# pytorch/ao

Hardware: NVIDIA H100
Metric: tok/s Llama-3-8B int4-wo (tile_packed_to_4d, g=32) linear stack, decode (higher is better)
Workload: dtype int4 weights -> bf16 MMA (f32 accumulate)

## Files before the change

### ao_b200/csrc/int4_linear.cu

```cuda
#include <cuda_bf16.h>
#include <stdlib.h>

#include "common.h"
#include "ptx.cuh"
#include "ts_gemm.cuh"

namespace ao {
namespace int4k {

using tsg::KCHUNK;
using tsg::ROWS;

__device__ __forceinline__ uint32_t deq_pair(uint32_t magic_bits, __nv_bfloat162 s2, __nv_bfloat162 z2) {
  const __nv_bfloat162 c136 = __floats2bfloat162_rn(136.f, 136.f);
  __nv_bfloat162 v = *reinterpret_cast<__nv_bfloat162*>(&magic_bits);
  v = __hsub2(v, c136);
  v = __hfma2(v, s2, z2);
  return *reinterpret_cast<uint32_t*>(&v);
}

struct Int4Fmt {
  static constexpr bool SS = false;
  static constexpr bool DECODE_2CTA = true;
  static constexpr bool PROMOTE = false;
  static constexpr int X_ELEM_BYTES = 2;
  static constexpr int W_BYTES = ROWS * KCHUNK / 2;
  static constexpr int AUX_BYTES = 2048;
  static constexpr int EPI = tsg::EPI_FLOAT;
  static constexpr int ACC_EXP2 = 0;
  static constexpr int MAX_N_MMA = 128;
  static int make_maps(const int32_t* qdata, const uint16_t* sz, int N, int K, int g, CUtensorMap* tm_w,
                       CUtensorMap* tm_sz) {
    const int KT = K / 128;
    {
      const uint64_t dims[3] = {32, (uint64_t)4 * KT, (uint64_t)N / 8};
      const uint64_t str[2] = {128, (uint64_t)KT * 512};
      const uint32_t box[3] = {32, 4, 16};
      int rc = make_tmap(tm_w, CU_TENSOR_MAP_DATA_TYPE_INT32, 3, qdata, dims, str, box, CU_TENSOR_MAP_SWIZZLE_128B);
      if (rc) return rc;
    }
    const int gpc = g <= 128 ? 128 / g : 1;
    const uint64_t dims[2] = {(uint64_t)N, (uint64_t)K / g};
    const uint64_t str[1] = {(uint64_t)N * 4};
    const uint32_t box[2] = {128, (uint32_t)gpc};
    return make_tmap(tm_sz, CU_TENSOR_MAP_DATA_TYPE_UINT32, 2, sz, dims, str, box, CU_TENSOR_MAP_SWIZZLE_NONE);
  }
  __device__ static __forceinline__ uint32_t w_tx_bytes(const tsg::Params& p) {
    const int gpc = p.group_size <= KCHUNK ? KCHUNK / p.group_size : 1;
    return W_BYTES + gpc * 512;
  }
  __device__ static __forceinline__ void issue_w(const CUtensorMap* tm_w, const CUtensorMap* tm_sz,
                                                 const tsg::Params& p, uint8_t* w_dst, uint8_t* aux_dst,
                                                 uint64_t* bar, int n_tile, int kc, uint64_t policy) {
    tma_load_3d(w_dst, tm_w, bar, 0, 4 * kc, n_tile * (ROWS / 8), policy);
    tma_load_2d(aux_dst, tm_sz, bar, n_tile * ROWS, (kc * KCHUNK) / p.group_size, policy);
  }
  struct Raw {
    uint4 v[2];
    uint32_t sz[2][4];
  };
  __device__ static __forceinline__ void load(const tsg::Params& p, uint32_t w_smem, uint32_t aux_smem, int row_lo,
                                              int lane, Raw& raw) {
    const int gshift = p.group_size == 32 ? 0 : (p.group_size == 64 ? 1 : 2);
#pragma unroll
    for (int h = 0; h < 2; ++h) {
      const int r = row_lo + 8 * h;
      const uint32_t off = (uint32_t)(r >> 3) * 512u + (uint32_t)lane * 16u;
      raw.v[h] = tsg::lds128(w_smem + (off ^ (((off >> 7) & 7) << 4)));
#pragma unroll
      for (int w = 0; w < 4; ++w) raw.sz[h][w] = tsg::lds32(aux_smem + r * 4 + (w >> gshift) * 512);
    }
  }
  __device__ static __forceinline__ void frag(const tsg::Params&, const Raw& raw, int kk, uint32_t (&a)[4]) {
    uint32_t magic = 0x43004300u;
    asm volatile("" : "+r"(magic));
    const int wd = kk >> 1, e0 = 2 * (kk & 1);
#pragma unroll
    for (int h = 0; h < 2; ++h) {
      const uint32_t sz = raw.sz[h][wd];
      const uint32_t s_bits = __byte_perm(sz, sz, 0x1010);
      const uint32_t z_bits = __byte_perm(sz, sz, 0x3232);
      const __nv_bfloat162 s2 = *reinterpret_cast<const __nv_bfloat162*>(&s_bits);
      const __nv_bfloat162 z2 = *reinterpret_cast<const __nv_bfloat162*>(&z_bits);
      const uint32_t word = wd == 0 ? raw.v[h].x : wd == 1 ? raw.v[h].y : wd == 2 ? raw.v[h].z : raw.v[h].w;
#pragma unroll
      for (int e = 0; e < 2; ++e) {
        uint32_t m;
        asm("lop3.b32 %0, %1, %2, %3, 0xEA;" : "=r"(m) : "r"(word >> (4 * (e0 + e))), "r"(0x000F000Fu), "r"(magic));
        a[h + 2 * e] = deq_pair(m, s2, z2);
      }
    }
  }
};

template <int MT>
__global__ void int4_linear_simple_kernel(const __nv_bfloat16* __restrict__ x,
                                          const int32_t* __restrict__ qdata,
                                          const __nv_bfloat16* __restrict__ sz,
                                          const __nv_bfloat16* __restrict__ bias,
                                          __nv_bfloat16* __restrict__ y, int M, int N, int N_out,
                                          int K, int g, int ldx) {
  const int warp = threadIdx.x >> 5, lane = threadIdx.x & 31;
  const int n = blockIdx.x * 8 + warp;
  const int m0 = blockIdx.y * MT;
  if (n >= N) return;
  const int KT = K / 128;
  float acc[MT];
#pragma unroll
  for (int m = 0; m < MT; ++m) acc[m] = 0.f;
  for (int ko = lane; ko < KT; ko += 32) {
    const uint4* wp = reinterpret_cast<const uint4*>(qdata + (((size_t)(n >> 3) * KT + ko) * 32 + (n & 7) * 4) * 4);
    for (int tq = 0; tq < 4; ++tq) {
      const uint4 v = wp[tq];
      const uint32_t words[4] = {v.x, v.y, v.z, v.w};
#pragma unroll
      for (int wd = 0; wd < 4; ++wd) {
#pragma unroll
        for (int e = 0; e < 4; ++e) {
#pragma unroll
          for (int h = 0; h < 2; ++h) {
            const int k = ko * 128 + 32 * wd + 2 * tq + 8 * e + h;
            const int q = (words[wd] >> (4 * e + 16 * h)) & 15;
            const size_t gi = ((size_t)(k / g) * N + n) * 2;
            const __nv_bfloat16 wv = __hfma(__int2bfloat16_rn(q - 8), sz[gi], sz[gi + 1]);
            const float wf = __bfloat162float(wv);
#pragma unroll
            for (int m = 0; m < MT; ++m)
              if (m0 + m < M) acc[m] += __bfloat162float(x[(size_t)(m0 + m) * ldx + k]) * wf;
          }
        }
      }
    }
  }
#pragma unroll
  for (int m = 0; m < MT; ++m) {
    float v = acc[m];
    for (int o = 16; o > 0; o >>= 1) v += __shfl_xor_sync(0xffffffffu, v, o);
    if (lane == 0 && m0 + m < M && n < N_out)
      y[(size_t)(m0 + m) * N_out + n] = __float2bfloat16_rn(v + (bias ? __bfloat162float(bias[n]) : 0.f));
  }
}

// ... 48 lines not shown
```

### ao_b200/csrc/lowp_linear.cu

```cuda
#include <cuda_bf16.h>
#include <cuda_fp8.h>
#include <stdlib.h>

#include <type_traits>

#include "common.h"
#include "nvfp4_fmt.cuh"
#include "ptx.cuh"
#include "streamk.cuh"
#include "ts_gemm.cuh"

namespace ao {
namespace lowp {

enum Kind { KIND_I8 = 0, KIND_F8 = 1, KIND_MXF8 = 2, KIND_NVF4 = 3 };

using tsg::KCHUNK;
using tsg::ROWS;

static int kmajor_byte_map(const uint8_t* wq, int N, int K, CUtensorMap* tm) {
  const uint64_t dims[2] = {(uint64_t)K, (uint64_t)N};
  const uint64_t str[1] = {(uint64_t)K};
  const uint32_t box[2] = {KCHUNK, ROWS};
  return make_tmap(tm, CU_TENSOR_MAP_DATA_TYPE_UINT8, 2, wq, dims, str, box, CU_TENSOR_MAP_SWIZZLE_128B);
// ... 13 lines not shown
  static int make_maps(const uint8_t* wq, int N, int K, CUtensorMap* tm_w, CUtensorMap* tm_aux) {
    if (int rc = kmajor_byte_map(wq, N, K, tm_w)) return rc;
    *tm_aux = *tm_w;
    return AO_OK;
  }
  __device__ static __forceinline__ uint32_t w_tx_bytes(const tsg::Params&) { return W_BYTES; }
  __device__ static __forceinline__ void issue_w(const CUtensorMap* tm_w, const CUtensorMap*, const tsg::Params&,
                                                 uint8_t* w_dst, uint8_t*, uint64_t* bar, int n_tile, int kc,
                                                 uint64_t policy) {
    tma_load_2d(w_dst, tm_w, bar, kc * KCHUNK, n_tile * ROWS, policy);
  }
  template <int N_MMA>
  __device__ static __forceinline__ void mma(uint32_t (&acc)[N_MMA / 2], uint32_t w_s, uint32_t x_s, int wg,
                                             uint32_t scale_d) {
#pragma unroll
    for (int kk = 0; kk < 4; ++kk) {
      const uint64_t ad = wgmma_desc_k_sw128(w_s + wg * (64 * 128) + kk * 32);
      const uint64_t bd = wgmma_desc_k_sw128(x_s + kk * 32);
      if (KIND == KIND_I8) Wgmma<N_MMA>::ss_s8(acc, ad, bd, kk == 0 ? scale_d : 1u);
      else Wgmma<N_MMA>::ss_e4m3(acc, ad, bd, kk == 0 ? scale_d : 1u);
    }
  }
};

__device__ __forceinline__ float e8m0_to_f32(uint32_t e) {
  return __uint_as_float(e == 0xFFu ? 0x7FC00000u : (e ? e << 23 : 0x00400000u));
}

struct Mxfp8Fmt {
  static constexpr bool SS = false;
  static constexpr bool DECODE_2CTA = false;
  static constexpr bool PROMOTE = false;
  static constexpr int X_ELEM_BYTES = 2;
  static constexpr int W_BYTES = ROWS * KCHUNK;
  static constexpr int AUX_BYTES = 512;
  static constexpr int EPI = tsg::EPI_FLOAT;
  static constexpr int ACC_EXP2 = 0;
  static constexpr int MAX_N_MMA = 128;
  static int make_maps(const uint8_t* wq, const uint8_t* w_sf, int N, int K, CUtensorMap* tm_w, CUtensorMap* tm_sf) {
    if (int rc = kmajor_byte_map(wq, N, K, tm_w)) return rc;
    const uint64_t dims[2] = {128, (uint64_t)ceil_div(N, ROWS) * (uint64_t)ceil_div(K / 32, 4)};
    const uint64_t str[1] = {512};
    const uint32_t box[2] = {128, 1};
    return make_tmap(tm_sf, CU_TENSOR_MAP_DATA_TYPE_UINT32, 2, w_sf, dims, str, box, CU_TENSOR_MAP_SWIZZLE_NONE);
  }
  __device__ static __forceinline__ uint32_t w_tx_bytes(const tsg::Params&) { return W_BYTES + AUX_BYTES; }
  __device__ static __forceinline__ void issue_w(const CUtensorMap* tm_w, const CUtensorMap* tm_sf, const tsg::Params& p,
                                                 uint8_t* w_dst, uint8_t* aux_dst, uint64_t* bar, int n_tile, int kc,
                                                 uint64_t policy) {
    tma_load_2d(w_dst, tm_w, bar, kc * KCHUNK, n_tile * ROWS, policy);
    tma_load_2d(aux_dst, tm_sf, bar, 0, n_tile * p.aux_col_blocks + kc, policy);
  }
  struct Raw {
    uint32_t v[2][8];
    uint32_t sc[2];
  };
  __device__ static __forceinline__ void load(const tsg::Params&, uint32_t w_smem, uint32_t aux_smem, int row_lo, int lane,
                                              Raw& raw) {
    const int t = lane & 3;
#pragma unroll
    for (int h = 0; h < 2; ++h) {
      const int r = row_lo + 8 * h;
      raw.sc[h] = tsg::lds32(aux_smem + (uint32_t)(r & 31) * 16u + (uint32_t)(r >> 5) * 4u);
#pragma unroll
      for (int kk = 0; kk < 8; ++kk) {
        const uint32_t a = w_smem + (uint32_t)r * 128u + ((uint32_t)(kk ^ (r & 7)) << 4) + 2 * t;
        raw.v[h][kk] = tsg::lds16(a) | (tsg::lds16(a + 8) << 16);
      }
    }
  }
  __device__ static __forceinline__ uint32_t deq(uint32_t pair, float s) {
    const __half2_raw hr = __nv_cvt_fp8x2_to_halfraw2((__nv_fp8x2_storage_t)pair, __NV_E4M3);
    const float2 f = __half22float2(*reinterpret_cast<const __half2*>(&hr));
    __nv_bfloat162 b = __floats2bfloat162_rn(f.x * s, f.y * s);
    return *reinterpret_cast<uint32_t*>(&b);
  }
  __device__ static __forceinline__ void frag(const tsg::Params&, const Raw& raw, int kk, uint32_t (&a)[4]) {
#pragma unroll
    for (int h = 0; h < 2; ++h) {
      const float s = e8m0_to_f32((raw.sc[h] >> (8 * (kk >> 1))) & 0xFFu);
      a[h] = deq(raw.v[h][kk] & 0xFFFFu, s);
      a[h + 2] = deq(raw.v[h][kk] >> 16, s);
    }
  }
};

template <int KIND>
__global__ void __launch_bounds__(256) dequant_act_kernel(const uint8_t* __restrict__ xq, const uint8_t* __restrict__ x_sf,
                                                          int m0, int rows, int K, int sf_col_blocks,
                                                          __nv_bfloat16* __restrict__ out) {
  pdl_launch_dependents();
  pdl_wait();
  const int per_row = K / 16;
  const long long idx = (long long)blockIdx.x * blockDim.x + threadIdx.x;
  if (idx >= (long long)rows * per_row) return;
  const int mr = (int)(idx / per_row), k0 = (int)(idx % per_row) * 16, m = m0 + mr;
  const int kb = KIND == KIND_NVF4 ? k0 / 16 : k0 / 32;
  const size_t tile = (size_t)(m / 128) * sf_col_blocks + kb / 4;
  const uint32_t sbyte = x_sf[tile * 512 + (m % 32) * 16 + ((m % 128) / 32) * 4 + kb % 4];
  __nv_bfloat16 o[16];
  if (KIND == KIND_NVF4) {
    const __half_raw sh = __nv_cvt_fp8_to_halfraw((__nv_fp8_storage_t)sbyte, __NV_E4M3);
    const float s = __half2float(*reinterpret_cast<const __half*>(&sh));
    const uint2 v = *reinterpret_cast<const uint2*>(xq + (size_t)m * (K / 2) + k0 / 2);
    const float lut[8] = {0.f, 0.5f, 1.f, 1.5f, 2.f, 3.f, 4.f, 6.f};
#pragma unroll
    for (int j = 0; j < 16; ++j) {
      const uint32_t nib = ((j < 8 ? v.x : v.y) >> (4 * (j & 7))) & 0xFu;
      const float x = lut[nib & 7] * s;
      o[j] = __float2bfloat16_rn(nib & 8 ? -x : x);
    }
  } else {
    const float s = e8m0_to_f32(sbyte);
    const uint4 v = *reinterpret_cast<const uint4*>(xq + (size_t)m * K + k0);
    const uint32_t w[4] = {v.x, v.y, v.z, v.w};
#pragma unroll
    for (int j = 0; j < 8; ++j) {
      const __half2_raw hr = __nv_cvt_fp8x2_to_halfraw2((__nv_fp8x2_storage_t)(w[j >> 1] >> (16 * (j & 1))), __NV_E4M3);
      const float2 f = __half22float2(*reinterpret_cast<const __half2*>(&hr));
      o[2 * j] = __float2bfloat16_rn(f.x * s);
      o[2 * j + 1] = __float2bfloat16_rn(f.y * s);
    }
  }
  uint4* dst = reinterpret_cast<uint4*>(out + (size_t)mr * K + k0);
  dst[0] = reinterpret_cast<const uint4*>(o)[0];
  dst[1] = reinterpret_cast<const uint4*>(o)[1];
}

template <int KIND>
static int rowwise(const uint8_t* xq, const float* x_scale, int M, int K, const uint8_t* wq, const float* w_scale, int N,
                   const uint16_t* bias, uint16_t* y, int32_t* i32_out, void* ws, size_t ws_bytes, void* stream) {
  using Fmt = SsFmt<KIND>;
  CUtensorMap tm_w, tm_aux;
  if (int rc = Fmt::make_maps(wq, N, K, &tm_w, &tm_aux)) return rc;
  tsg::Params p{};
// ... 143 lines not shown
```

### ao_b200/csrc/nvfp4_fmt.cuh

```cuda
#pragma once
#include <cuda_bf16.h>

#include "ptx.cuh"
#include "ts_gemm.cuh"

namespace ao {
namespace nvf4w {

struct Nvfp4Fmt {
  static constexpr bool SS = false;
  static constexpr bool DECODE_2CTA = false;
  static constexpr bool PROMOTE = false;
  static constexpr int X_ELEM_BYTES = 2;
  static constexpr int W_BYTES = tsg::ROWS * tsg::KCHUNK / 2;
  static constexpr int AUX_BYTES = 1024;
  static constexpr int EPI = tsg::EPI_FLOAT;
  static constexpr int ACC_EXP2 = 60;
  static constexpr int MAX_N_MMA = 128;
  static int make_maps(const uint8_t* wq, const uint8_t* w_sf, int N, int K, CUtensorMap* tm_w, CUtensorMap* tm_sf) {
    {
      const uint64_t dims[2] = {(uint64_t)K / 2, (uint64_t)N};
      const uint64_t str[1] = {(uint64_t)K / 2};
      const uint32_t box[2] = {64, 128};
      int rc = make_tmap(tm_w, CU_TENSOR_MAP_DATA_TYPE_UINT8, 2, wq, dims, str, box, CU_TENSOR_MAP_SWIZZLE_64B);
      if (rc) return rc;
    }
    const uint64_t dims[2] = {128, (uint64_t)ceil_div(N, tsg::ROWS) * (uint64_t)ceil_div(K / 16, 4)};
    const uint64_t str[1] = {512};
    const uint32_t box[2] = {128, 2};
    return make_tmap(tm_sf, CU_TENSOR_MAP_DATA_TYPE_UINT32, 2, w_sf, dims, str, box, CU_TENSOR_MAP_SWIZZLE_NONE);
  }
  __device__ static __forceinline__ uint32_t w_tx_bytes(const tsg::Params&) { return W_BYTES + AUX_BYTES; }
  __device__ static __forceinline__ void issue_w(const CUtensorMap* tm_w, const CUtensorMap* tm_sf, const tsg::Params& p,
                                                 uint8_t* w_dst, uint8_t* aux_dst, uint64_t* bar, int n_tile, int kc,
                                                 uint64_t policy) {
    tma_load_2d(w_dst, tm_w, bar, kc * 64, n_tile * tsg::ROWS, policy);
    tma_load_2d(aux_dst, tm_sf, bar, 0, n_tile * p.aux_col_blocks + kc * 2, policy);
  }
  struct Raw {
    uint2 v[2][8];
    uint32_t s2[2][4];
  };
  __device__ static __forceinline__ void load(const tsg::Params&, uint32_t w_smem, uint32_t aux_smem, int row_lo, int,
                                              Raw& raw) {
#pragma unroll
    for (int h = 0; h < 2; ++h) {
      const int r = row_lo + 8 * h;
      const uint32_t sc_off = (uint32_t)(r & 31) * 16u + (uint32_t)(r >> 5) * 4u;
      const uint32_t sc[2] = {tsg::lds32(aux_smem + sc_off), tsg::lds32(aux_smem + 512 + sc_off)};
#pragma unroll
      for (int j = 0; j < 4; ++j) {
        const uint32_t bits = __byte_perm(sc[j >> 1], 0u, (j & 1) ? 0x4342u : 0x4140u) << 4;
        __nv_bfloat162 s2 = *reinterpret_cast<const __nv_bfloat162*>(&bits);
        s2 = __hmul2(__hmul2(s2, __nv_bfloat162(__ushort_as_bfloat16(0x7F00), __ushort_as_bfloat16(0x7F00))),
                     __nv_bfloat162(__ushort_as_bfloat16(0x5D00), __ushort_as_bfloat16(0x5D00)));
        raw.s2[h][j] = *reinterpret_cast<const uint32_t*>(&s2);
      }
#pragma unroll
      for (int kk = 0; kk < 8; ++kk) {
        const uint32_t off = (uint32_t)r * 64u + kk * 8;
        raw.v[h][kk] = tsg::lds64(w_smem + (off ^ (((off >> 7) & 3) << 4)));
      }
    }
  }
  __device__ static __forceinline__ uint32_t deq(uint32_t byte, __nv_bfloat162 s2) {
    const uint32_t hh = (byte | (byte << 12)) & 0x000F000Fu;
    const uint32_t bits = (hh * 0x1040u) & 0x81C081C0u;
    __nv_bfloat162 x = *reinterpret_cast<const __nv_bfloat162*>(&bits);
    x = __hmul2(x, s2);
    return *reinterpret_cast<uint32_t*>(&x);
  }
  __device__ static __forceinline__ void frag(const tsg::Params&, const Raw& raw, int kk, uint32_t (&a)[4]) {
    const int t = threadIdx.x & 3;
#pragma unroll
    for (int h = 0; h < 2; ++h) {
      const uint32_t s_bits = __byte_perm(raw.s2[h][kk >> 1], 0u, (kk & 1) ? 0x3232u : 0x1010u);
      const __nv_bfloat162 s2 = *reinterpret_cast<const __nv_bfloat162*>(&s_bits);
      a[h] = deq((raw.v[h][kk].x >> (8 * t)) & 0xFFu, s2);
      a[h + 2] = deq((raw.v[h][kk].y >> (8 * t)) & 0xFFu, s2);
    }
  }
};

}
}
```

### ao_b200/csrc/ptx.cuh

```cuda
#pragma once
#include <cuda_runtime.h>
#include <stdint.h>

namespace ao {

__device__ __forceinline__ uint32_t smem_u32(const void* p) {
  return static_cast<uint32_t>(__cvta_generic_to_shared(p));
}

__device__ __forceinline__ bool elect_one() {
  uint32_t pred = 0;
  asm volatile(
      "{\n\t.reg .pred P;\n\t"
      "elect.sync _|P, 0xffffffff;\n\t"
      "selp.b32 %0, 1, 0, P;\n\t}\n"
      : "=r"(pred));
  return pred != 0;
}

__device__ __forceinline__ void mbar_init(uint64_t* bar, uint32_t count) {
  asm volatile("mbarrier.init.shared::cta.b64 [%0], %1;" ::"r"(smem_u32(bar)), "r"(count));
}
__device__ __forceinline__ void fence_barrier_init() {
  asm volatile("fence.mbarrier_init.release.cluster;" ::: "memory");
}
__device__ __forceinline__ void fence_proxy_async() {
  asm volatile("fence.proxy.async.shared::cta;" ::: "memory");
}
__device__ __forceinline__ void mbar_arrive(uint64_t* bar) {
  asm volatile("mbarrier.arrive.shared::cta.b64 _, [%0];" ::"r"(smem_u32(bar)) : "memory");
}
__device__ __forceinline__ void mbar_expect_tx(uint64_t* bar, uint32_t bytes) {
  asm volatile("mbarrier.arrive.expect_tx.shared::cta.b64 _, [%0], %1;" ::"r"(smem_u32(bar)),
               "r"(bytes)
               : "memory");
}
__device__ __forceinline__ bool mbar_try_wait(uint64_t* bar, uint32_t parity) {
  uint32_t ok;
  asm volatile(
      "{\n\t.reg .pred P;\n\t"
      "mbarrier.try_wait.parity.shared::cta.b64 P, [%1], %2;\n\t"
      "selp.b32 %0, 1, 0, P;\n\t}\n"
      : "=r"(ok)
      : "r"(smem_u32(bar)), "r"(parity)
      : "memory");
  return ok != 0;
}
__device__ __forceinline__ void mbar_wait(uint64_t* bar, uint32_t parity) {
  while (!mbar_try_wait(bar, parity)) {
  }
}

__device__ __forceinline__ void tma_prefetch_desc(const void* tmap) {
  asm volatile("prefetch.tensormap [%0];" ::"l"(tmap) : "memory");
}
__device__ __forceinline__ uint64_t policy_evict_first() {
  uint64_t p;
  asm volatile("createpolicy.fractional.L2::evict_first.b64 %0, 1.0;" : "=l"(p));
  return p;
}
__device__ __forceinline__ uint64_t policy_evict_last() {
  uint64_t p;
  asm volatile("createpolicy.fractional.L2::evict_last.b64 %0, 1.0;" : "=l"(p));
  return p;
}
__device__ __forceinline__ void tma_load_2d(void* dst, const void* tmap, uint64_t* bar, int c0,
                                            int c1, uint64_t policy) {
  asm volatile(
      "cp.async.bulk.tensor.2d.shared::cluster.global.mbarrier::complete_tx::bytes.L2::cache_hint"
      " [%0], [%1, {%3, %4}], [%2], %5;" ::"r"(smem_u32(dst)),
      "l"(tmap), "r"(smem_u32(bar)), "r"(c0), "r"(c1), "l"(policy)
      : "memory");
}
__device__ __forceinline__ void tma_load_3d(void* dst, const void* tmap, uint64_t* bar, int c0,
                                            int c1, int c2, uint64_t policy) {
  asm volatile(
      "cp.async.bulk.tensor.3d.shared::cluster.global.mbarrier::complete_tx::bytes.L2::cache_hint"
      " [%0], [%1, {%3, %4, %5}], [%2], %6;" ::"r"(smem_u32(dst)),
      "l"(tmap), "r"(smem_u32(bar)), "r"(c0), "r"(c1), "r"(c2), "l"(policy)
      : "memory");
}

__device__ __forceinline__ void pdl_wait() { asm volatile("griddepcontrol.wait;" ::: "memory"); }
__device__ __forceinline__ void pdl_launch_dependents() {
  asm volatile("griddepcontrol.launch_dependents;" ::: "memory");
}

template <int N>
__device__ __forceinline__ void setmaxnreg_dec() { asm volatile("setmaxnreg.dec.sync.aligned.u32 %0;" ::"n"(N)); }
template <int N>
__device__ __forceinline__ void setmaxnreg_inc() { asm volatile("setmaxnreg.inc.sync.aligned.u32 %0;" ::"n"(N)); }

__device__ __forceinline__ uint64_t wgmma_desc_k_sw128(uint32_t smem_addr) {
  uint64_t d = 0;
  d |= (uint64_t)((smem_addr & 0x3FFFF) >> 4);
  d |= (uint64_t)1 << 16;
  d |= (uint64_t)(1024 >> 4) << 32;
  d |= (uint64_t)1 << 62;
  return d;
}

}
```

### ao_b200/csrc/ts_gemm.cuh

```cuda
#pragma once
#include <cuda_bf16.h>

#include "common.h"
#include "ptx.cuh"
#include "streamk.cuh"
#include "wgmma.cuh"

namespace ao {
namespace tsg {

using streamk::ROWS;
constexpr int KCHUNK = 128;
constexpr int NUM_THREADS = 384;
constexpr int CONSUMER_WARPS = 8;
constexpr int MAX_STAGES = 12;
constexpr int SMEM_PER_SM = 228 * 1024, SMEM_RESERVED_PER_CTA = 1024;
template <class Fmt, int N_MMA>
constexpr int ctas_per_sm() { return N_MMA <= 32 && Fmt::DECODE_2CTA ? 2 : 1; }
constexpr int PRODUCER_REGS = 24, CONSUMER_REGS = 104;

enum Epi { EPI_FLOAT = 0, EPI_I8 = 1, EPI_F8 = 2 };

struct Params {
  const __nv_bfloat16* bias;
// ... 8 lines not shown
  unsigned int* ws_flag;
  int M, N, N_out, K, group_size;
  int n_tiles, m_blocks, KT;
  int aux_col_blocks;
};

template <class Fmt, int N_MMA>
struct Cfg {
  static constexpr int X_BYTES = N_MMA * KCHUNK * Fmt::X_ELEM_BYTES;
  static constexpr int X_ATOMS = Fmt::X_ELEM_BYTES;
  static constexpr int AUX_SLOT = (Fmt::AUX_BYTES + 1023) & ~1023;
  static constexpr int STAGE_BYTES = Fmt::W_BYTES + AUX_SLOT + X_BYTES;
  static constexpr int CTAS = ctas_per_sm<Fmt, N_MMA>();
  static constexpr int STAGES_FIT = CTAS == 1 ? 200 * 1024 / STAGE_BYTES
                                              : (SMEM_PER_SM / 2 - SMEM_RESERVED_PER_CTA - 1024) / (STAGE_BYTES + 24);
  static constexpr int STAGES = STAGES_FIT > MAX_STAGES ? MAX_STAGES : STAGES_FIT;
  static_assert(STAGES >= 2, "stage does not fit");
  static constexpr int BAR_OFF = STAGES * STAGE_BYTES;
  static constexpr int BAR_BYTES = 3 * STAGES * 8;
  static constexpr size_t SMEM_BYTES = (size_t)BAR_OFF + BAR_BYTES + 1024;
  static_assert(CTAS * (SMEM_BYTES + SMEM_RESERVED_PER_CTA) <= SMEM_PER_SM, "CTAs per SM do not fit");
};

__device__ __forceinline__ uint4 lds128(uint32_t addr) {
  uint4 v;
  asm volatile("ld.shared.v4.u32 {%0,%1,%2,%3}, [%4];" : "=r"(v.x), "=r"(v.y), "=r"(v.z), "=r"(v.w) : "r"(addr));
  return v;
}
__device__ __forceinline__ uint2 lds64(uint32_t addr) {
  uint2 v;
  asm volatile("ld.shared.v2.u32 {%0,%1}, [%2];" : "=r"(v.x), "=r"(v.y) : "r"(addr));
  return v;
}
__device__ __forceinline__ uint32_t lds32(uint32_t addr) {
  uint32_t v;
  asm volatile("ld.shared.u32 %0, [%1];" : "=r"(v) : "r"(addr));
  return v;
}
__device__ __forceinline__ uint32_t lds16(uint32_t addr) {
  unsigned short v;
  asm volatile("ld.shared.u16 %0, [%1];" : "=h"(v) : "r"(addr));
  return v;
}

template <class Fmt, int N_MMA>
__global__ void __launch_bounds__(NUM_THREADS, ctas_per_sm<Fmt, N_MMA>())
ts_gemm_kernel(const __grid_constant__ CUtensorMap tm_w, const __grid_constant__ CUtensorMap tm_aux,
               const __grid_constant__ CUtensorMap tm_x, const Params p) {
  using C = Cfg<Fmt, N_MMA>;
  using MMA = Wgmma<N_MMA>;
  constexpr int S = C::STAGES;
  constexpr int NACC = N_MMA / 2;
  extern __shared__ uint8_t smem_raw[];
  uint8_t* smem = reinterpret_cast<uint8_t*>((reinterpret_cast<uintptr_t>(smem_raw) + 1023) & ~uintptr_t(1023));
  uint64_t* bars = reinterpret_cast<uint64_t*>(smem + C::BAR_OFF);
  uint64_t* wfull = bars;
  uint64_t* xfull = wfull + S;
  uint64_t* sempty = xfull + S;

  const int warp = __shfl_sync(0xffffffffu, (int)(threadIdx.x >> 5), 0), lane = threadIdx.x & 31;
  const int wgi = __shfl_sync(0xffffffffu, (int)(threadIdx.x >> 7), 0);
  const int G = gridDim.x, b = blockIdx.x;
  const long long U = (long long)p.n_tiles * p.m_blocks * p.KT;
  const int u0 = streamk::unit_begin(b, U, G), u1 = streamk::unit_begin(b + 1, U, G);
  const int nunits = u1 - u0;
  const streamk::Walk walk(u0, nunits, p.KT);
  auto tile_of = [&](int i) { return (u0 + i) / p.KT; };
  auto kc_of = [&](int i) { return (u0 + i) % p.KT; };
  auto stage = [&](int s) { return smem + (size_t)s * C::STAGE_BYTES; };

  if (threadIdx.x == 0) {
    for (int i = 0; i < S; ++i) {
      mbar_init(&wfull[i], 1);
      mbar_init(&xfull[i], 1);
      mbar_init(&sempty[i], CONSUMER_WARPS);
    }
    fence_barrier_init();
  }
  if (warp == 0 && lane == 0) {
    tma_prefetch_desc(&tm_w);
    tma_prefetch_desc(&tm_aux);
    tma_prefetch_desc(&tm_x);
  }
  __syncthreads();
  pdl_launch_dependents();

  const int seg_last = walk.nseg - 1;
  const bool last_is_owner = walk.seg_kind(seg_last) == streamk::SEG_OWNER;

  if (wgi == 0) {
    if constexpr (C::CTAS > 1) setmaxnreg_dec<PRODUCER_REGS>();
    if (warp != 0) goto done;
    const uint64_t pol_w = policy_evict_first();
    const uint64_t pol_x = policy_evict_last();
    auto issue_w = [&](int i) {
      const int s = i % S;
      uint8_t* st = stage(s);
      mbar_expect_tx(&wfull[s], Fmt::w_tx_bytes(p));
      Fmt::issue_w(&tm_w, &tm_aux, p, st, st + Fmt::W_BYTES, &wfull[s], tile_of(i) % p.n_tiles, kc_of(i), pol_w);
    };
    auto issue_x = [&](int i) {
      const int s = i % S;
      uint8_t* xs = stage(s) + Fmt::W_BYTES + C::AUX_SLOT;
      const int m0 = (tile_of(i) / p.n_tiles) * N_MMA;
      mbar_expect_tx(&xfull[s], C::X_BYTES);
#pragma unroll
      for (int a = 0; a < C::X_ATOMS; ++a)
        tma_load_2d(xs + a * (N_MMA * 128), &tm_x, &xfull[s], kc_of(i) * KCHUNK + a * (KCHUNK / C::X_ATOMS), m0, pol_x);
    };
    const int pre = nunits < S ? nunits : S;
    for (int i = 0; i < pre; ++i) {
      if (elect_one()) issue_w(i);
      __syncwarp();
    }
    pdl_wait();
    for (int i = 0; i < pre; ++i) {
      if (elect_one()) issue_x(i);
      __syncwarp();
    }
    for (int i = S; i < nunits; ++i) {
      mbar_wait(&sempty[i % S], ((i / S) & 1) ^ 1);
      if (elect_one()) {
        issue_w(i);
        issue_x(i);
      }
      __syncwarp();
    }
  } else {
    if constexpr (C::CTAS > 1) setmaxnreg_inc<CONSUMER_REGS>();
    const int wg = wgi - 1, wq = warp & 3;
    const int g = lane >> 2, t = lane & 3;
    const int row_lo = wg * 64 + wq * 16 + g;
    pdl_wait();

    uint32_t acc[NACC];
    uint32_t a[8][4];
    int pending = -1;
    auto release = [&](int s) {
      __syncwarp();
      if (lane == 0) mbar_arrive(&sempty[s]);
    };

    auto epilogue = [&](int seg, uint32_t (&v)[NACC]) {
      const int tile = walk.seg_tile(seg);
      const int kind = walk.seg_kind(seg);
      const int n_tile = tile % p.n_tiles, m_blk = tile / p.n_tiles;
      const int m0 = m_blk * N_MMA;
      if (kind == streamk::SEG_CONTRIB) {
        uint32_t* slot = reinterpret_cast<uint32_t*>(p.ws_partial) + (size_t)b * (N_MMA * ROWS);
#pragma unroll
        for (int q = 0; q < NACC / 4; ++q)
#pragma unroll
          for (int h = 0; h < 2; ++h)
#pragma unroll
            for (int c = 0; c < 2; ++c) {
              const int col = 8 * q + 2 * t + c, r = row_lo + 8 * h;
              if (m0 + col < p.M) __stcg(&slot[col * ROWS + r], v[4 * q + 2 * h + c]);
            }
        asm volatile("bar.sync 1, 256;" ::: "memory");
        if (warp == 4 && lane == 0) streamk::st_release_u32(p.ws_flag + b, 1u);
        return;
      }
      if (kind == streamk::SEG_OWNER) {
        const int b_last = streamk::cta_of_unit((long long)tile * p.KT + p.KT - 1, U, G);
        if (warp == 4) streamk::wait_flags(p.ws_flag + b + 1, b_last - b, lane);
        asm volatile("bar.sync 1, 256;" ::: "memory");
        constexpr int GB = NACC <= 8 ? 4 : (NACC <= 16 ? 2 : 1);
#pragma unroll 1
        for (int c = b + 1; c <= b_last && GB == 1; ++c) {
          const uint32_t* slot = reinterpret_cast<const uint32_t*>(p.ws_partial) + (size_t)c * (N_MMA * ROWS);
#pragma unroll
          for (int q = 0; q < NACC / 4; ++q) {
            if (q % 2 == 0 && m0 + 8 * q >= p.M) break;
#pragma unroll
            for (int h = 0; h < 2; ++h)
#pragma unroll
              for (int cc = 0; cc < 2; ++cc) {
                const int col = 8 * q + 2 * t + cc, r = row_lo + 8 * h, j = 4 * q + 2 * h + cc;
                if (m0 + col < p.M) {
                  const uint32_t o = __ldcg(slot + col * ROWS + r);
                  if constexpr (Fmt::EPI == EPI_I8) v[j] = (uint32_t)((int32_t)v[j] + (int32_t)o);
                  else v[j] = __float_as_uint(__uint_as_float(v[j]) + __uint_as_float(o));
                }
              }
          }
        }
#pragma unroll 1
        for (int c0 = b + 1; c0 <= b_last && GB > 1; c0 += GB) {
          uint32_t o[GB][NACC];
#pragma unroll
          for (int gi = 0; gi < GB; ++gi) {
            if (c0 + gi > b_last) break;
            const uint32_t* slot = reinterpret_cast<const uint32_t*>(p.ws_partial) + (size_t)(c0 + gi) * (N_MMA * ROWS);
#pragma unroll
            for (int q = 0; q < NACC / 4; ++q)
#pragma unroll
              for (int h = 0; h < 2; ++h)
#pragma unroll
                for (int cc = 0; cc < 2; ++cc) {
                  const int col = 8 * q + 2 * t + cc, r = row_lo + 8 * h, j = 4 * q + 2 * h + cc;
                  o[gi][j] = m0 + col < p.M ? __ldcg(slot + col * ROWS + r) : 0u;
                }
          }
#pragma unroll
          for (int gi = 0; gi < GB; ++gi) {
            if (c0 + gi > b_last) break;
#pragma unroll
            for (int q = 0; q < NACC / 4; ++q)
#pragma unroll
              for (int h = 0; h < 2; ++h)
#pragma unroll
                for (int cc = 0; cc < 2; ++cc) {
                  const int j = 4 * q + 2 * h + cc;
                  if constexpr (Fmt::EPI == EPI_I8) v[j] = (uint32_t)((int32_t)v[j] + (int32_t)o[gi][j]);
                  else v[j] = __float_as_uint(__uint_as_float(v[j]) + __uint_as_float(o[gi][j]));
                }
          }
        }
      }
#pragma unroll
      for (int h = 0; h < 2; ++h) {
        const int n = n_tile * ROWS + row_lo + 8 * h;
        if (n >= p.N_out) continue;
        const float bias = p.bias ? __bfloat162float(p.bias[n]) : 0.f;
        float osc = 1.f, sw = 1.f;
        if constexpr (Fmt::EPI == EPI_FLOAT) {
          osc = (p.out_scale ? (p.out_scale_per_row ? p.out_scale[n] : *p.out_scale) : 1.f);
          if (p.out_scale2) osc *= *p.out_scale2;
          osc *= __int_as_float((127 + Fmt::ACC_EXP2) << 23);
        } else {
          sw = p.w_scale ? p.w_scale[n] : 1.f;
        }
#pragma unroll
        for (int q = 0; q < NACC / 4; ++q)
#pragma unroll
          for (int c = 0; c < 2; ++c) {
            const int m = m0 + 8 * q + 2 * t + c;
            if (m >= p.M) continue;
            const uint32_t raw = v[4 * q + 2 * h + c];
            __nv_bfloat16* dst = p.y ? p.y + (size_t)m * p.N_out + n : nullptr;
            if constexpr (Fmt::EPI == EPI_FLOAT) {
              float x = __uint_as_float(raw);
              if (p.row_scale) x *= p.row_scale[m];
              *dst = __float2bfloat16_rn(x * osc + bias);
            } else if constexpr (Fmt::EPI == EPI_I8) {
              if (p.i32_out) {
                p.i32_out[(size_t)m * p.N_out + n] = (int32_t)raw;
              } else {
                const float x = __bfloat162float(__float2bfloat16_rn((float)(int32_t)raw * p.row_scale[m]));
                *dst = __float2bfloat16_rn(x * sw + bias);
              }
            } else {
              *dst = __float2bfloat16_rn(__uint_as_float(raw) * (p.row_scale[m] * sw) + bias);
            }
          }
      }
    };

    int i = 0;
    for (int seg = 0; seg < walk.nseg; ++seg) {
      const int cnt = walk.seg_count(seg);
      for (int c = 0; c < cnt; ++c, ++i) {
        const uint32_t scale_d = c > 0;
        const int s = i % S;
        const uint32_t ph = (i / S) & 1;
        uint8_t* st = stage(s);
        const uint32_t w_s = smem_u32(st), aux_s = w_s + Fmt::W_BYTES, x_s = aux_s + C::AUX_SLOT;
        mbar_wait(&wfull[s], ph);
        if constexpr (Fmt::PROMOTE) {
          mbar_wait(&xfull[s], ph);
          uint32_t part[NACC];
          wgmma_fence();
          Fmt::template mma<N_MMA>(part, w_s, x_s, wg, 0u);
          wgmma_commit();
          wgmma_wait<0>();
          wgmma_fence_operand(part);
          release(s);
#pragma unroll
          for (int j = 0; j < NACC; ++j)
            acc[j] = scale_d ? __float_as_uint(__uint_as_float(acc[j]) + __uint_as_float(part[j])) : part[j];
          continue;
        } else if constexpr (Fmt::SS) {
          mbar_wait(&xfull[s], ph);
          wgmma_fence_operand(acc);
          wgmma_fence();
          Fmt::template mma<N_MMA>(acc, w_s, x_s, wg, scale_d);
        } else {
          typename Fmt::Raw raw;
          Fmt::load(p, w_s, aux_s, row_lo, lane, raw);
          wgmma_wait<0>();
#pragma unroll
          for (int kk = 0; kk < 8; ++kk) wgmma_fence_operand(a[kk]);
          if (pending >= 0) release(pending);
          pending = -1;
#pragma unroll
          for (int kk = 0; kk < 4; ++kk) Fmt::frag(p, raw, kk, a[kk]);
          mbar_wait(&xfull[s], ph);
          wgmma_fence_operand(acc);
#pragma unroll
          for (int half = 0; half < 2; ++half) {
            if (half == 1) {
              uint32_t(&rw)[sizeof(raw) / 4] = *reinterpret_cast<uint32_t(*)[sizeof(raw) / 4]>(&raw);
              wgmma_fence_operand(rw);
#pragma unroll
              for (int kk = 4; kk < 8; ++kk) Fmt::frag(p, raw, kk, a[kk]);
            }
            wgmma_fence();
#pragma unroll
            for (int kk = 4 * half; kk < 4 * half + 4; ++kk) {
              const uint64_t bd = wgmma_desc_k_sw128(x_s + (kk >> 2) * (N_MMA * 128) + (kk & 3) * 32);
              MMA::ra_bf16(acc, a[kk], bd, kk == 0 ? scale_d : 1u);
            }
          }
        }
        wgmma_commit();
        wgmma_fence_operand(acc);
        wgmma_wait<1>();
        if (pending >= 0) release(pending);
        pending = s;
      }
      wgmma_wait<0>();
      wgmma_fence_operand(acc);
      if (pending >= 0) release(pending);
      pending = -1;
      epilogue(seg, acc);
    }
  }

done:
  __syncthreads();
  if (last_is_owner && warp == 4) {
    const int b_last = streamk::cta_of_unit((long long)walk.seg_tile(seg_last) * p.KT + p.KT - 1, U, G);
    for (int c = b + 1 + lane; c <= b_last; c += 32) p.ws_flag[c] = 0u;
  }
}

template <class Fmt, int N_MMA>
inline int launch_gemm(Params& p, const CUtensorMap& tm_w, const CUtensorMap& tm_aux, const void* x, int ldx,
                       void* ws, size_t ws_bytes, const char* what, cudaStream_t stream) {
  using C = Cfg<Fmt, N_MMA>;
  CUtensorMap tm_x;
  {
    const uint64_t dims[2] = {(uint64_t)p.K, (uint64_t)p.M};
    const uint64_t str[1] = {(uint64_t)ldx * Fmt::X_ELEM_BYTES};
    const uint32_t box[2] = {128 / Fmt::X_ELEM_BYTES, N_MMA};
    int rc = make_tmap(&tm_x, Fmt::X_ELEM_BYTES == 2 ? CU_TENSOR_MAP_DATA_TYPE_BFLOAT16 : CU_TENSOR_MAP_DATA_TYPE_UINT8,
                       2, x, dims, str, box, CU_TENSOR_MAP_SWIZZLE_128B);
    if (rc) return rc;
  }
  p.m_blocks = ceil_div(p.M, N_MMA);
  const long long units = (long long)p.n_tiles * p.m_blocks * p.KT;
  int grid = sm_count();
  constexpr int min_units = 4;
  if (units / min_units < grid) grid = units / min_units > 0 ? (int)(units / min_units) : 1;
  if (const int forced = streamk_ctas_override()) {
    const int cap = units < sm_count() ? (int)units : sm_count();
    grid = forced < 1 ? 1 : (forced > cap ? cap : forced);
  }
  const size_t need = streamk::WS_PARTIAL_OFF + (size_t)grid * N_MMA * ROWS * 4;
  if (!ws || ws_bytes < need || (size_t)grid * 4 > streamk::WS_FLAGS_BYTES)
    return fail(AO_ERR_WORKSPACE, "%s: workspace too small (%zu < %zu)", what, ws_bytes, need);
  p.ws_flag = reinterpret_cast<unsigned int*>(ws);
  p.ws_partial = reinterpret_cast<float*>(reinterpret_cast<uint8_t*>(ws) + streamk::WS_PARTIAL_OFF);
  auto kern = ts_gemm_kernel<Fmt, N_MMA>;
  AO_CUDA_CHECK(ensure_dynamic_smem(reinterpret_cast<const void*>(kern), C::SMEM_BYTES));
  AO_CUDA_CHECK(launch(kern, dim3(grid), dim3(NUM_THREADS), C::SMEM_BYTES, stream, pdl_enabled(), tm_w, tm_aux, tm_x, p));
  return AO_OK;
}

template <class Fmt>
inline int run(Params& p, const CUtensorMap& tm_w, const CUtensorMap& tm_aux, const void* x, int ldx, void* ws,
               size_t ws_bytes, const char* what, cudaStream_t stream) {
  static_assert(Fmt::MAX_N_MMA == 64 || Fmt::MAX_N_MMA == 128, "token tile");
  p.n_tiles = ceil_div(p.N_out, ROWS);
  p.KT = ceil_div(p.K, KCHUNK);
  if (p.M <= 16) return launch_gemm<Fmt, 16>(p, tm_w, tm_aux, x, ldx, ws, ws_bytes, what, stream);
  if (p.M <= 32) return launch_gemm<Fmt, 32>(p, tm_w, tm_aux, x, ldx, ws, ws_bytes, what, stream);
// ... 7 lines not shown
```

Before: 9705.

## Split per-stage weight load and dequant into two halves with per-half wgmma commit

Restructures the register-A mainloop so each stage loads and dequantizes weights in two halves. Each half has its own wgmma commit and waits only on the previous group, so dequant of the second half overlaps the first half's MMAs and register pressure drops. It also hoists dequant constants, replaces the modulo/divide stage indexing with an incrementing ring index and phase bit, precomputes descriptor low words and barrier addresses, and uses a predicated mbarrier arrive. The release logic is reworked to release the previous stage, which carries some risk of ordering or hazard bugs across segments.

Result: faster. 9942, median of 6 (+2.4%).

```diff
diff --git a/ao_b200/csrc/int4_linear.cu b/ao_b200/csrc/int4_linear.cu
--- a/ao_b200/csrc/int4_linear.cu
+++ b/ao_b200/csrc/int4_linear.cu
@@ -11,8 +11,8 @@
 using tsg::KCHUNK;
 using tsg::ROWS;
 
-__device__ __forceinline__ uint32_t deq_pair(uint32_t magic_bits, __nv_bfloat162 s2, __nv_bfloat162 z2) {
-  const __nv_bfloat162 c136 = __floats2bfloat162_rn(136.f, 136.f);
+__device__ __forceinline__ uint32_t deq_pair(uint32_t magic_bits, __nv_bfloat162 c136, __nv_bfloat162 s2,
+                                             __nv_bfloat162 z2) {
   __nv_bfloat162 v = *reinterpret_cast<__nv_bfloat162*>(&magic_bits);
   v = __hsub2(v, c136);
   v = __hfma2(v, s2, z2);
@@ -56,25 +56,30 @@
     tma_load_2d(aux_dst, tm_sz, bar, n_tile * ROWS, (kc * KCHUNK) / p.group_size, policy);
   }
   struct Raw {
-    uint4 v[2];
-    uint32_t sz[2][4];
+    uint2 v[2];
+    uint32_t sz[2][2];
   };
   __device__ static __forceinline__ void load(const tsg::Params& p, uint32_t w_smem, uint32_t aux_smem, int row_lo,
-                                              int lane, Raw& raw) {
+                                              int lane, int half, Raw& raw) {
     const int gshift = p.group_size == 32 ? 0 : (p.group_size == 64 ? 1 : 2);
 #pragma unroll
     for (int h = 0; h < 2; ++h) {
       const int r = row_lo + 8 * h;
       const uint32_t off = (uint32_t)(r >> 3) * 512u + (uint32_t)lane * 16u;
-      raw.v[h] = tsg::lds128(w_smem + (off ^ (((off >> 7) & 7) << 4)));
+      raw.v[h] = tsg::lds64(w_smem + (off ^ (((off >> 7) & 7) << 4)) + 8 * half);
 #pragma unroll
-      for (int w = 0; w < 4; ++w) raw.sz[h][w] = tsg::lds32(aux_smem + r * 4 + (w >> gshift) * 512);
+      for (int w = 0; w < 2; ++w) raw.sz[h][w] = tsg::lds32(aux_smem + r * 4 + ((2 * half + w) >> gshift) * 512);
     }
   }
-  __device__ static __forceinline__ void frag(const tsg::Params&, const Raw& raw, int kk, uint32_t (&a)[4]) {
-    uint32_t magic = 0x43004300u;
-    asm volatile("" : "+r"(magic));
-    const int wd = kk >> 1, e0 = 2 * (kk & 1);
+  struct Consts {
+    uint32_t magic;
+    __nv_bfloat162 c136;
+  };
+  __device__ static __forceinline__ Consts consts(const tsg::Params&) {
+    return Consts{0x43004300u, __nv_bfloat162(__ushort_as_bfloat16(0x4308), __ushort_as_bfloat16(0x4308))};
+  }
+  __device__ static __forceinline__ void frag(const Consts& k, const Raw& raw, int kk, uint32_t (&a)[4]) {
+    const int wd = (kk >> 1) & 1, e0 = 2 * (kk & 1);
 #pragma unroll
     for (int h = 0; h < 2; ++h) {
       const uint32_t sz = raw.sz[h][wd];
@@ -82,12 +87,12 @@
       const uint32_t z_bits = __byte_perm(sz, sz, 0x3232);
       const __nv_bfloat162 s2 = *reinterpret_cast<const __nv_bfloat162*>(&s_bits);
       const __nv_bfloat162 z2 = *reinterpret_cast<const __nv_bfloat162*>(&z_bits);
-      const uint32_t word = wd == 0 ? raw.v[h].x : wd == 1 ? raw.v[h].y : wd == 2 ? raw.v[h].z : raw.v[h].w;
+      const uint32_t word = wd == 0 ? raw.v[h].x : raw.v[h].y;
 #pragma unroll
       for (int e = 0; e < 2; ++e) {
         uint32_t m;
-        asm("lop3.b32 %0, %1, %2, %3, 0xEA;" : "=r"(m) : "r"(word >> (4 * (e0 + e))), "r"(0x000F000Fu), "r"(magic));
-        a[h + 2 * e] = deq_pair(m, s2, z2);
+        asm("lop3.b32 %0, %1, %2, %3, 0xEA;" : "=r"(m) : "r"(word >> (4 * (e0 + e))), "r"(0x000F000Fu), "r"(k.magic));
+        a[h + 2 * e] = deq_pair(m, k.c136, s2, z2);
       }
     }
   }
diff --git a/ao_b200/csrc/lowp_linear.cu b/ao_b200/csrc/lowp_linear.cu
--- a/ao_b200/csrc/lowp_linear.cu
+++ b/ao_b200/csrc/lowp_linear.cu
@@ -89,20 +89,21 @@
     tma_load_2d(aux_dst, tm_sf, bar, 0, n_tile * p.aux_col_blocks + kc, policy);
   }
   struct Raw {
-    uint32_t v[2][8];
+    uint32_t v[2][4];
     uint32_t sc[2];
   };
   __device__ static __forceinline__ void load(const tsg::Params&, uint32_t w_smem, uint32_t aux_smem, int row_lo, int lane,
-                                              Raw& raw) {
+                                              int half, Raw& raw) {
     const int t = lane & 3;
 #pragma unroll
     for (int h = 0; h < 2; ++h) {
       const int r = row_lo + 8 * h;
       raw.sc[h] = tsg::lds32(aux_smem + (uint32_t)(r & 31) * 16u + (uint32_t)(r >> 5) * 4u);
 #pragma unroll
-      for (int kk = 0; kk < 8; ++kk) {
+      for (int kq = 0; kq < 4; ++kq) {
+        const int kk = 4 * half + kq;
         const uint32_t a = w_smem + (uint32_t)r * 128u + ((uint32_t)(kk ^ (r & 7)) << 4) + 2 * t;
-        raw.v[h][kk] = tsg::lds16(a) | (tsg::lds16(a + 8) << 16);
+        raw.v[h][kq] = tsg::lds16(a) | (tsg::lds16(a + 8) << 16);
       }
     }
   }
@@ -112,12 +113,14 @@
     __nv_bfloat162 b = __floats2bfloat162_rn(f.x * s, f.y * s);
     return *reinterpret_cast<uint32_t*>(&b);
   }
-  __device__ static __forceinline__ void frag(const tsg::Params&, const Raw& raw, int kk, uint32_t (&a)[4]) {
+  struct Consts {};
+  __device__ static __forceinline__ Consts consts(const tsg::Params&) { return {}; }
+  __device__ static __forceinline__ void frag(const Consts&, const Raw& raw, int kk, uint32_t (&a)[4]) {
 #pragma unroll
     for (int h = 0; h < 2; ++h) {
       const float s = e8m0_to_f32((raw.sc[h] >> (8 * (kk >> 1))) & 0xFFu);
-      a[h] = deq(raw.v[h][kk] & 0xFFFFu, s);
-      a[h + 2] = deq(raw.v[h][kk] >> 16, s);
+      a[h] = deq(raw.v[h][kk & 3] & 0xFFFFu, s);
+      a[h + 2] = deq(raw.v[h][kk & 3] >> 16, s);
     }
   }
 };
diff --git a/ao_b200/csrc/nvfp4_fmt.cuh b/ao_b200/csrc/nvfp4_fmt.cuh
--- a/ao_b200/csrc/nvfp4_fmt.cuh
+++ b/ao_b200/csrc/nvfp4_fmt.cuh
@@ -38,28 +38,28 @@
     tma_load_2d(aux_dst, tm_sf, bar, 0, n_tile * p.aux_col_blocks + kc * 2, policy);
   }
   struct Raw {
-    uint2 v[2][8];
-    uint32_t s2[2][4];
+    uint2 v[2][4];
+    uint32_t s2[2][2];
   };
   __device__ static __forceinline__ void load(const tsg::Params&, uint32_t w_smem, uint32_t aux_smem, int row_lo, int,
-                                              Raw& raw) {
+                                              int half, Raw& raw) {
 #pragma unroll
     for (int h = 0; h < 2; ++h) {
       const int r = row_lo + 8 * h;
       const uint32_t sc_off = (uint32_t)(r & 31) * 16u + (uint32_t)(r >> 5) * 4u;
-      const uint32_t sc[2] = {tsg::lds32(aux_smem + sc_off), tsg::lds32(aux_smem + 512 + sc_off)};
+      const uint32_t sc = tsg::lds32(aux_smem + 512 * half + sc_off);
 #pragma unroll
-      for (int j = 0; j < 4; ++j) {
-        const uint32_t bits = __byte_perm(sc[j >> 1], 0u, (j & 1) ? 0x4342u : 0x4140u) << 4;
+      for (int j = 0; j < 2; ++j) {
+        const uint32_t bits = __byte_perm(sc, 0u, j ? 0x4342u : 0x4140u) << 4;
         __nv_bfloat162 s2 = *reinterpret_cast<const __nv_bfloat162*>(&bits);
         s2 = __hmul2(__hmul2(s2, __nv_bfloat162(__ushort_as_bfloat16(0x7F00), __ushort_as_bfloat16(0x7F00))),
                      __nv_bfloat162(__ushort_as_bfloat16(0x5D00), __ushort_as_bfloat16(0x5D00)));
         raw.s2[h][j] = *reinterpret_cast<const uint32_t*>(&s2);
       }
 #pragma unroll
-      for (int kk = 0; kk < 8; ++kk) {
-        const uint32_t off = (uint32_t)r * 64u + kk * 8;
-        raw.v[h][kk] = tsg::lds64(w_smem + (off ^ (((off >> 7) & 3) << 4)));
+      for (int kq = 0; kq < 4; ++kq) {
+        const uint32_t off = (uint32_t)r * 64u + (4 * half + kq) * 8;
+        raw.v[h][kq] = tsg::lds64(w_smem + (off ^ (((off >> 7) & 3) << 4)));
       }
     }
   }
@@ -70,14 +70,16 @@
     x = __hmul2(x, s2);
     return *reinterpret_cast<uint32_t*>(&x);
   }
-  __device__ static __forceinline__ void frag(const tsg::Params&, const Raw& raw, int kk, uint32_t (&a)[4]) {
-    const int t = threadIdx.x & 3;
+  struct Consts {};
+  __device__ static __forceinline__ Consts consts(const tsg::Params&) { return {}; }
+  __device__ static __forceinline__ void frag(const Consts&, const Raw& raw, int kk, uint32_t (&a)[4]) {
+    const int t = threadIdx.x & 3, kq = kk & 3;
 #pragma unroll
     for (int h = 0; h < 2; ++h) {
-      const uint32_t s_bits = __byte_perm(raw.s2[h][kk >> 1], 0u, (kk & 1) ? 0x3232u : 0x1010u);
+      const uint32_t s_bits = __byte_perm(raw.s2[h][kq >> 1], 0u, (kk & 1) ? 0x3232u : 0x1010u);
       const __nv_bfloat162 s2 = *reinterpret_cast<const __nv_bfloat162*>(&s_bits);
-      a[h] = deq((raw.v[h][kk].x >> (8 * t)) & 0xFFu, s2);
-      a[h + 2] = deq((raw.v[h][kk].y >> (8 * t)) & 0xFFu, s2);
+      a[h] = deq((raw.v[h][kq].x >> (8 * t)) & 0xFFu, s2);
+      a[h + 2] = deq((raw.v[h][kq].y >> (8 * t)) & 0xFFu, s2);
     }
   }
 };
diff --git a/ao_b200/csrc/ptx.cuh b/ao_b200/csrc/ptx.cuh
--- a/ao_b200/csrc/ptx.cuh
+++ b/ao_b200/csrc/ptx.cuh
@@ -27,29 +27,38 @@
 __device__ __forceinline__ void fence_proxy_async() {
   asm volatile("fence.proxy.async.shared::cta;" ::: "memory");
 }
-__device__ __forceinline__ void mbar_arrive(uint64_t* bar) {
-  asm volatile("mbarrier.arrive.shared::cta.b64 _, [%0];" ::"r"(smem_u32(bar)) : "memory");
+__device__ __forceinline__ void mbar_arrive(uint32_t bar) {
+  asm volatile("mbarrier.arrive.shared::cta.b64 _, [%0];" ::"r"(bar) : "memory");
+}
+__device__ __forceinline__ void mbar_arrive(uint64_t* bar) { mbar_arrive(smem_u32(bar)); }
+__device__ __forceinline__ void mbar_arrive_if(bool pred, uint32_t bar) {
+  asm volatile(
+      "{\n\t.reg .pred P;\n\t"
+      "setp.ne.b32 P, %1, 0;\n\t"
+      "@P mbarrier.arrive.shared::cta.b64 _, [%0];\n\t}\n" ::"r"(bar), "r"((uint32_t)pred)
+      : "memory");
 }
 __device__ __forceinline__ void mbar_expect_tx(uint64_t* bar, uint32_t bytes) {
   asm volatile("mbarrier.arrive.expect_tx.shared::cta.b64 _, [%0], %1;" ::"r"(smem_u32(bar)),
                "r"(bytes)
                : "memory");
 }
-__device__ __forceinline__ bool mbar_try_wait(uint64_t* bar, uint32_t parity) {
+__device__ __forceinline__ bool mbar_try_wait(uint32_t bar, uint32_t parity) {
   uint32_t ok;
   asm volatile(
       "{\n\t.reg .pred P;\n\t"
       "mbarrier.try_wait.parity.shared::cta.b64 P, [%1], %2;\n\t"
       "selp.b32 %0, 1, 0, P;\n\t}\n"
       : "=r"(ok)
-      : "r"(smem_u32(bar)), "r"(parity)
+      : "r"(bar), "r"(parity)
       : "memory");
   return ok != 0;
 }
-__device__ __forceinline__ void mbar_wait(uint64_t* bar, uint32_t parity) {
+__device__ __forceinline__ void mbar_wait(uint32_t bar, uint32_t parity) {
   while (!mbar_try_wait(bar, parity)) {
   }
 }
+__device__ __forceinline__ void mbar_wait(uint64_t* bar, uint32_t parity) { mbar_wait(smem_u32(bar), parity); }
 
 __device__ __forceinline__ void tma_prefetch_desc(const void* tmap) {
   asm volatile("prefetch.tensormap [%0];" ::"l"(tmap) : "memory");
@@ -91,13 +100,17 @@
 template <int N>
 __device__ __forceinline__ void setmaxnreg_inc() { asm volatile("setmaxnreg.inc.sync.aligned.u32 %0;" ::"n"(N)); }
 
+__device__ __forceinline__ uint32_t wgmma_desc_lo_k_sw128(uint32_t smem_addr) {
+  return ((smem_addr & 0x3FFFF) >> 4)
+         | 1u << 16;
+}
+__device__ __forceinline__ uint64_t wgmma_desc_k_sw128_lo(uint32_t lo) {
+  return (uint64_t)((1024 >> 4)
+                    | 1u << 30)
+             << 32 | lo;
+}
 __device__ __forceinline__ uint64_t wgmma_desc_k_sw128(uint32_t smem_addr) {
-  uint64_t d = 0;
-  d |= (uint64_t)((smem_addr & 0x3FFFF) >> 4);
-  d |= (uint64_t)1 << 16;
-  d |= (uint64_t)(1024 >> 4) << 32;
-  d |= (uint64_t)1 << 62;
-  return d;
+  return wgmma_desc_k_sw128_lo(wgmma_desc_lo_k_sw128(smem_addr));
 }
 
 }
diff --git a/ao_b200/csrc/ts_gemm.cuh b/ao_b200/csrc/ts_gemm.cuh
--- a/ao_b200/csrc/ts_gemm.cuh
+++ b/ao_b200/csrc/ts_gemm.cuh
@@ -84,7 +84,8 @@
   constexpr int S = C::STAGES;
   constexpr int NACC = N_MMA / 2;
   extern __shared__ uint8_t smem_raw[];
-  uint8_t* smem = reinterpret_cast<uint8_t*>((reinterpret_cast<uintptr_t>(smem_raw) + 1023) & ~uintptr_t(1023));
+  const uint32_t smem_s = (smem_u32(smem_raw) + 1023) & ~1023u;
+  uint8_t* smem = smem_raw + (smem_s - smem_u32(smem_raw));
   uint64_t* bars = reinterpret_cast<uint64_t*>(smem + C::BAR_OFF);
   uint64_t* wfull = bars;
   uint64_t* xfull = wfull + S;
@@ -167,16 +168,16 @@
 
     uint32_t acc[NACC];
     uint32_t a[8][4];
-    int pending = -1;
-    auto release = [&](int s) {
+    const uint32_t sempty_s = smem_s + C::BAR_OFF + 16 * S;
+    auto release = [&](bool pending, int s) {
       __syncwarp();
-      if (lane == 0) mbar_arrive(&sempty[s]);
+      mbar_arrive_if(lane == 0 && pending, sempty_s + 8 * s);
     };
 
     auto epilogue = [&](int seg, uint32_t (&v)[NACC]) {
       const int tile = walk.seg_tile(seg);
       const int kind = walk.seg_kind(seg);
-      const int n_tile = tile % p.n_tiles, m_blk = tile / p.n_tiles;
+      const int m_blk = tile / p.n_tiles;
       const int m0 = m_blk * N_MMA;
       if (kind == streamk::SEG_CONTRIB) {
         uint32_t* slot = reinterpret_cast<uint32_t*>(p.ws_partial) + (size_t)b * (N_MMA * ROWS);
@@ -250,6 +251,7 @@
           }
         }
       }
+      const int n_tile = tile - m_blk * p.n_tiles;
 #pragma unroll
       for (int h = 0; h < 2; ++h) {
         const int n = n_tile * ROWS + row_lo + 8 * h;
@@ -289,72 +291,72 @@
       }
     };
 
-    int i = 0;
+    const uint32_t ring = smem_s, wfull_s = ring + C::BAR_OFF, xfull_s = wfull_s + 8 * S;
+    const uint32_t xdesc0 = wgmma_desc_lo_k_sw128(ring + Fmt::W_BYTES + C::AUX_SLOT);
+    const auto consts = [&] {
+      if constexpr (Fmt::SS) return 0;
+      else return Fmt::consts(p);
+    }();
+    int s = 0;
+    uint32_t ph = 0;
+    auto prev = [&] { return s == 0 ? S - 1 : s - 1; };
     for (int seg = 0; seg < walk.nseg; ++seg) {
       const int cnt = walk.seg_count(seg);
-      for (int c = 0; c < cnt; ++c, ++i) {
+      for (int c = 0; c < cnt; ++c, s = s + 1 == S ? 0 : s + 1, ph ^= s == 0) {
         const uint32_t scale_d = c > 0;
-        const int s = i % S;
-        const uint32_t ph = (i / S) & 1;
-        uint8_t* st = stage(s);
-        const uint32_t w_s = smem_u32(st), aux_s = w_s + Fmt::W_BYTES, x_s = aux_s + C::AUX_SLOT;
-        mbar_wait(&wfull[s], ph);
+        const uint32_t w_s = ring + s * C::STAGE_BYTES, aux_s = w_s + Fmt::W_BYTES, x_s = aux_s + C::AUX_SLOT;
+        mbar_wait(wfull_s + 8 * s, ph);
         if constexpr (Fmt::PROMOTE) {
-          mbar_wait(&xfull[s], ph);
+          mbar_wait(xfull_s + 8 * s, ph);
           uint32_t part[NACC];
           wgmma_fence();
           Fmt::template mma<N_MMA>(part, w_s, x_s, wg, 0u);
           wgmma_commit();
           wgmma_wait<0>();
           wgmma_fence_operand(part);
-          release(s);
+          release(true, s);
 #pragma unroll
           for (int j = 0; j < NACC; ++j)
             acc[j] = scale_d ? __float_as_uint(__uint_as_float(acc[j]) + __uint_as_float(part[j])) : part[j];
-          continue;
         } else if constexpr (Fmt::SS) {
-          mbar_wait(&xfull[s], ph);
+          mbar_wait(xfull_s + 8 * s, ph);
           wgmma_fence_operand(acc);
           wgmma_fence();
           Fmt::template mma<N_MMA>(acc, w_s, x_s, wg, scale_d);
+          wgmma_commit();
+          wgmma_fence_operand(acc);
+          wgmma_wait<1>();
+          release(c > 0, prev());
         } else {
-          typename Fmt::Raw raw;
-          Fmt::load(p, w_s, aux_s, row_lo, lane, raw);
-          wgmma_wait<0>();
-#pragma unroll
-          for (int kk = 0; kk < 8; ++kk) wgmma_fence_operand(a[kk]);
-          if (pending >= 0) release(pending);
-          pending = -1;
-#pragma unroll
-          for (int kk = 0; kk < 4; ++kk) Fmt::frag(p, raw, kk, a[kk]);
-          mbar_wait(&xfull[s], ph);
-          wgmma_fence_operand(acc);
-#pragma unroll
-          for (int half = 0; half < 2; ++half) {
-            if (half == 1) {
-              uint32_t(&rw)[sizeof(raw) / 4] = *reinterpret_cast<uint32_t(*)[sizeof(raw) / 4]>(&raw);
-              wgmma_fence_operand(rw);
-#pragma unroll
-              for (int kk = 4; kk < 8; ++kk) Fmt::frag(p, raw, kk, a[kk]);
+          const uint32_t xd = xdesc0 + s * (C::STAGE_BYTES >> 4);
+          auto half = [&](int h) {
+            typename Fmt::Raw raw;
+            Fmt::load(p, w_s, aux_s, row_lo, lane, h, raw);
+            wgmma_wait<1>();
+#pragma unroll
+            for (int kk = 4 * h; kk < 4 * h + 4; ++kk) wgmma_fence_operand(a[kk]);
+            if (h == 1) release(c > 0, prev());
+#pragma unroll
+            for (int kk = 4 * h; kk < 4 * h + 4; ++kk) Fmt::frag(consts, raw, kk, a[kk]);
+            if (h == 0) {
+              mbar_wait(xfull_s + 8 * s, ph);
+              wgmma_fence_operand(acc);
             }
             wgmma_fence();
 #pragma unroll
-            for (int kk = 4 * half; kk < 4 * half + 4; ++kk) {
-              const uint64_t bd = wgmma_desc_k_sw128(x_s + (kk >> 2) * (N_MMA * 128) + (kk & 3) * 32);
-              MMA::ra_bf16(acc, a[kk], bd, kk == 0 ? scale_d : 1u);
-            }
-          }
+            for (int kk = 4 * h; kk < 4 * h + 4; ++kk)
+              MMA::ra_bf16(acc, a[kk], wgmma_desc_k_sw128_lo(xd + (((kk >> 2) * (N_MMA * 128) + (kk & 3) * 32) >> 4)),
+                           kk == 0 ? scale_d : 1u);
+            wgmma_commit();
+          };
+          half(0);
+          half(1);
+          wgmma_fence_operand(acc);
         }
-        wgmma_commit();
-        wgmma_fence_operand(acc);
-        wgmma_wait<1>();
-        if (pending >= 0) release(pending);
-        pending = s;
       }
       wgmma_wait<0>();
       wgmma_fence_operand(acc);
-      if (pending >= 0) release(pending);
-      pending = -1;
+      release(cnt > 0 && !Fmt::PROMOTE, prev());
       epilogue(seg, acc);
     }
   }
```
